# usamireko/WFL-ASR

Hardware: AMD Instinct MI355X
Metric: audio_seconds_labeled_per_sec_per_node (higher is better)
Workload: dtype bf16; 1 GPU; BASELINE configs[1]: openai/whisper-base + 2 Conformer blocks, 16 x 30 s clips per GPU; clips_per_gpu=16, frames_per_clip=1500, tags=141, parallelism=clip-sharded dp1, launch=eager, batches_in_flight=2

## Files before the change

include/wfl_asr.h:

```cpp
#ifndef WFL_ASR_H
#define WFL_ASR_H

#include <stdint.h>

#ifdef __cplusplus
extern "C" {
#endif

typedef struct wfl_model wfl_model;

#define WFL_ENC_WHISPER 0
#define WFL_ENC_WAVLM 1
#define WFL_ENC_NONE 2

#define WFL_ABI_VERSION 2

typedef struct wfl_arch {
  int32_t abi_version;
  int32_t encoder_type;
  int32_t d_model;
  int32_t enc_layers;
  int32_t enc_heads;
  int32_t enc_ffn;
  int32_t n_mels;
// ... 45 lines not shown

int32_t wfl_set_average_languages(wfl_model* m, const int32_t* ids_host, int32_t n);

int32_t wfl_num_frames(const wfl_model* m, int32_t L);
int64_t wfl_workspace_bytes(const wfl_model* m, int32_t B, int32_t L);

#define WFL_LANG_NONE 0
#define WFL_LANG_IDS 1
#define WFL_LANG_AVERAGE 2

int32_t wfl_forward(wfl_model* m, const float* wav, int64_t ldw, const int32_t* lens, int32_t B, int32_t L,
                    const int32_t* lang_id, int32_t lang_mode, float threshold, void* workspace,
                    int64_t workspace_bytes, int32_t* ids, int32_t* argmax, float* maxprob, float* offsets,
                    float* logits, float* hidden, int32_t* status, void* stream);

int32_t wfl_encode(wfl_model* m, const float* wav, int64_t ldw, const int32_t* lens, int32_t B, int32_t L, void* workspace,
                   int64_t workspace_bytes, float* hidden, void* stream);
int64_t wfl_head_workspace_bytes(const wfl_model* m, int32_t B, int32_t T);
int32_t wfl_head(wfl_model* m, const float* hidden, int32_t B, int32_t T, const int32_t* lang_id, int32_t lang_mode,
                 float threshold, void* workspace, int64_t workspace_bytes, int32_t* ids, int32_t* argmax, float* maxprob,
                 float* offsets, float* logits, int32_t* status, void* stream);

int32_t wfl_check(wfl_model* m, void* workspace, int64_t workspace_bytes, int32_t B, int32_t L, void* stream);


int32_t wfl_logmel(wfl_model* m, const float* wav, int64_t ldw, const int32_t* lens, int32_t B, int32_t L,
                   float* out, void* workspace, int64_t workspace_bytes, void* stream);

int32_t wfl_op_gemm(const void* A, int64_t lda, int32_t cin, int64_t tap_stride, const void* W, int32_t M, int32_t N,
                    int32_t K, int32_t n_valid, int32_t P, int32_t T, void* C, int64_t ldc, int64_t c_lead,
                    int32_t c_pitch, const float* bias, const void* res, int64_t ldres, float alpha, int32_t act,
                    int32_t glu, int32_t out_f32, void* stream);

int32_t wfl_op_gemm_split(const void* A_hi, const void* A_lo, int64_t lda, int32_t cin, int64_t tap_stride, const void* W3, int32_t M,
                          int32_t N, int32_t K, int32_t n_valid, int32_t P, int32_t T, void* C, void* C_lo, int64_t ldc,
                          int64_t c_lead, int32_t c_pitch, const float* bias, const void* res, const void* res_lo, int64_t ldres,
                          float alpha, int32_t act, int32_t glu, void* stream);

int32_t wfl_op_gemm_ln(const void* A, int64_t lda, const void* W, int32_t M, int32_t N, int32_t K, int32_t n_valid, int32_t P,
                       int32_t T, void* C, int64_t ldc, int64_t c_lead, int32_t c_pitch, const float* bias, const float* ln_s,
                       float ln_eps, int32_t act, void* stream);

int32_t wfl_op_attention(const void* QK, int64_t ldqk, int64_t lead, const void* V, int64_t ldv, void* O, int64_t ldo, int32_t B,
                         int32_t T, int32_t P, int32_t heads, int32_t d, void* stream);

int32_t wfl_op_attention_ex(const void* QK, const void* QK_lo, int64_t ldqk, int64_t lead, const void* V, const void* V_lo, int64_t ldv,
                            void* O, void* O_lo, int64_t ldo, int32_t B, int32_t T, int32_t P, int32_t heads, int32_t d, const float* bias,
                            const float* gate, const int32_t* clip_T, void* O8, void* O8_lo, int64_t ldo8, float o8_scale, int32_t* status,
                            void* stream);

int32_t wfl_op_relpos_table(const float* rel_emb, const int32_t* bucket_of_delta, int32_t max_t, int32_t heads, int32_t T, float* table,
                            void* stream);

int32_t wfl_op_relpos_gate(const void* x, const void* x_lo, int64_t ldx, int64_t lead, int32_t B, int32_t P, int32_t T, int32_t heads,
                           int32_t hd, const float* w8, const float* b8, const float* cst, float* gate, void* stream);

int32_t wfl_op_regroup(const void* x, int32_t d, int32_t groups, int32_t cpg, int64_t R, int64_t lead, int32_t B, int32_t P, int32_t T,
                       const int32_t* clip_T, void* xg, void* stream);

int32_t wfl_op_wav_stats(const float* wav, int64_t ldw, const int32_t* lens, int32_t B, int32_t L, double* stats, void* stream);

int32_t wfl_op_clip_frames(const int32_t* lens, int32_t B, int32_t L, int32_t n, const int32_t* kernel, const int32_t* stride,
                           int32_t min_len, int32_t* out, void* stream);

int64_t wfl_op_conv0_scratch_bytes(int32_t B, int32_t T0, int32_t C);
int32_t wfl_op_conv0(const float* wav, int64_t ldw, const int32_t* lens, int32_t B, int32_t L, const double* wstats, const float* w,
// ... 200 lines not shown
```

wfl-asr_amd/_lib.py:

```python
from __future__ import annotations

import ctypes as C
import os

import numpy as np

PKG = os.path.dirname(os.path.abspath(__file__))
LIB_PATH = os.environ.get("WFL_LIB_PATH") or os.path.join(PKG, "libwfl_asr_hip.so")
ABI_VERSION = 2


class WflArch(C.Structure):
    _fields_ = [
        ("abi_version", C.c_int32), ("encoder_type", C.c_int32), ("d_model", C.c_int32), ("enc_layers", C.c_int32),
        ("enc_heads", C.c_int32), ("enc_ffn", C.c_int32), ("n_mels", C.c_int32), ("max_positions", C.c_int32),
        ("num_classes", C.c_int32), ("o_id", C.c_int32), ("num_languages", C.c_int32), ("lang_emb_dim", C.c_int32),
        ("enable_bilstm", C.c_int32), ("bilstm_layers", C.c_int32), ("n_conformer", C.c_int32),
        ("conformer_heads", C.c_int32), ("conformer_ff_expansion", C.c_int32), ("conformer_kernel", C.c_int32),
        ("enable_dilated", C.c_int32), ("dilated_depth", C.c_int32), ("dilated_kernel", C.c_int32),
        ("wavlm_n_conv", C.c_int32), ("wavlm_conv_dim", C.c_int32 * 8), ("wavlm_conv_kernel", C.c_int32 * 8),
        ("wavlm_conv_stride", C.c_int32 * 8), ("wavlm_group_norm", C.c_int32), ("wavlm_conv_bias", C.c_int32),
        ("wavlm_stable_layer_norm", C.c_int32), ("wavlm_pos_conv_kernel", C.c_int32),
        ("wavlm_pos_conv_groups", C.c_int32), ("wavlm_num_buckets", C.c_int32), ("wavlm_max_distance", C.c_int32),
        ("wavlm_do_normalize", C.c_int32), ("fp8_weights", C.c_int32), ("mel_hop", C.c_int32), ("precision", C.c_int32), ("fp8_activations", C.c_int32),
        ("mel_sample_rate", C.c_int32), ("reserved", C.c_int32 * 5),
    ]


_P = C.c_void_p
_I = C.c_int32
_L = C.c_int64
_F = C.c_float

SIGNATURES = {
    "wfl_last_error": (C.c_char_p, []),
    "wfl_abi_version": (_I, []),
    "wfl_create": (_I, [C.POINTER(WflArch), C.POINTER(_P)]),
    "wfl_destroy": (None, [_P]),
    "wfl_load_tensor": (_I, [_P, C.c_char_p, _P, C.POINTER(_L), _I]),
    "wfl_finalize": (_I, [_P]),
    "wfl_num_frames": (_I, [_P, _I]),
    "wfl_workspace_bytes": (_L, [_P, _I, _I]),
    "wfl_device": (_I, [_P]),
    "wfl_set_average_languages": (_I, [_P, _P, _I]),
    "wfl_forward": (_I, [_P, _P, _L, _P, _I, _I, _P, _I, _F, _P, _L, _P, _P, _P, _P, _P, _P, _P, _P]),
    "wfl_encode": (_I, [_P, _P, _L, _P, _I, _I, _P, _L, _P, _P]),
    "wfl_head_workspace_bytes": (_L, [_P, _I, _I]),
    "wfl_head": (_I, [_P, _P, _I, _I, _P, _I, _F, _P, _L, _P, _P, _P, _P, _P, _P, _P]),
    "wfl_check": (_I, [_P, _P, _L, _I, _I, _P]),
    "wfl_logmel": (_I, [_P, _P, _L, _P, _I, _I, _P, _P, _L, _P]),
    "wfl_op_gemm": (_I, [_P, _L, _I, _L, _P, _I, _I, _I, _I, _I, _I, _P, _L, _L, _I, _P, _P, _L, _F, _I, _I, _I, _P]),
    "wfl_op_gemm_split": (_I, [_P, _P, _L, _I, _L, _P, _I, _I, _I, _I, _I, _I, _P, _P, _L, _L, _I, _P, _P, _P, _L, _F, _I, _I, _P]),
    "wfl_op_gemm_ln": (_I, [_P, _L, _P, _I, _I, _I, _I, _I, _I, _P, _L, _L, _I, _P, _P, _F, _I, _P]),
    "wfl_op_gemm_mx": (_I, [_P, _P, _L, _P, _P, _P, _F, _I, _I, _I, _I, _I, _P, _L, _L, _I, _P, _P, _P, _P, _F, _I, _P, _P, _L, _F, _P, _P]),
    "wfl_op_rows_fp8": (_I, [_P, _L, _P, _P, _P, _F, _L, _I, _I, _I, _I, _P, _P, _L, _P, _P]),
    "wfl_op_attention": (_I, [_P, _L, _L, _P, _L, _P, _L, _I, _I, _I, _I, _I, _P]),
    "wfl_op_attention_ex": (_I, [_P, _P, _L, _L, _P, _P, _L, _P, _P, _L, _I, _I, _I, _I, _I, _P, _P, _P, _P, _P, _L, _F, _P, _P]),
    "wfl_op_relpos_table": (_I, [_P, _P, _I, _I, _I, _P, _P]),
    "wfl_op_relpos_gate": (_I, [_P, _P, _L, _L, _I, _I, _I, _I, _I, _P, _P, _P, _P, _P]),
    "wfl_op_regroup": (_I, [_P, _I, _I, _I, _L, _L, _I, _I, _I, _P, _P, _P]),
    "wfl_op_wav_stats": (_I, [_P, _L, _P, _I, _I, _P, _P]),
    "wfl_op_clip_frames": (_I, [_P, _I, _I, _I, _P, _P, _I, _P, _P]),
    "wfl_op_conv0_scratch_bytes": (_L, [_I, _I, _I]),
    "wfl_op_conv0": (_I, [_P, _L, _P, _I, _I, _P, _P, _P, _P, _P, _I, _I, _P, _P, _L, _I, _I, _P, _L, _P]),
    "wfl_op_posconv": (_I, [_P, _L, _L, _I, _I, _I, _I, _I, _I, _P, _L, _P, _P, _P, _P, _P, _L, _P, _P]),
    "wfl_op_layernorm_act": (_I, [_P, _P, _L, _P, _P, _L, _P, _P, _F, _L, _I, _I, _I, _I, _I, _I, _P, _P]),
    "wfl_op_layernorm_pair": (_I, [_P, _P, _P, _P, _P, _P, _L, _P, _P, _P, _P, _F, _L, _I, _I, _I, _I, _I, _P, _P]),
    "wfl_op_layernorm": (_I, [_P, _L, _P, _L, _P, _P, _F, _L, _I, _I, _I, _I, _P]),
    "wfl_op_tag_decide": (_I, [_P, _L, _I, _I, _F, _I, _P, _P, _P, _P]),
    "wfl_host_median_filter": (_I, [_P, _I, _I, _P]),
    "wfl_host_decode_bio": (_I, [_P, _I, _P, _I, _P, _P, _I, C.c_double, _P, _P, _P, _I]),
    "wfl_host_merge_segments": (_I, [_P, _P, _P, _I, _I]),
    "wfl_host_format_lab": (_L, [_P, _P, _P, _I, _P, _I, _P, _L]),
    "wfl_host_load_wav": (_I, [C.c_char_p, _P, _L, _P, _P]),
    "wfl_host_load_wavs": (_I, [_P, _I, _P, _L, _L, _P, _P, _P, _I]),
    "wfl_host_load_wav_chunks": (_I, [C.c_char_p, _I, _L, _P, _L, _I, _P, _P, _P]),
    "wfl_host_read_pcm16": (_I, [_P, _I, _P, _L, _L, _P, _P, _P, _P, _I]),
    "wfl_resample_workspace_bytes": (_L, [_I, _I]),
    "wfl_resample_pcm16": (_I, [_P, _L, _P, _P, _I, _I, _I, _P, _L, _I, _P, _L, _P]),
    "wfl_boundary_workspace_bytes": (_L, [_I, _I]),
    "wfl_boundary_features": (_I, [_P, _L, _P, _I, _I, _P, _P, _P, _P, _P, _L, _P]),
    "wfl_align_workspace_bytes": (_L, [_P, _P, _I]),
    "wfl_align": (_I, [_P, _L, _I, _I, _P, _P, _P, _P, _P, _P, _I, _P, _L, _P, _P, _P, _P, _P]),
    "wfl_align_windowed": (_I, [_P, _L, _I, _I, _P, _P, _P, _P, _P, _P, _P, _I, _P, _L, _P, _P, _P, _P, _P]),
# ... 87 lines not shown
```

wfl-asr_amd/csrc/gemm_stream.hip:

```cpp
#include "common.h"
#include <cstdlib>
#include <cstring>
#include <type_traits>

#define SBK 32
#ifndef SNST
#define SNST 4
#endif

#ifndef SNCU
#define SNCU 256
#endif

typedef __attribute__((address_space(1))) const void* sgptr_t;
typedef __attribute__((address_space(3))) void* slptr_t;
typedef __attribute__((ext_vector_type(2))) __bf16 bf16x2;

static __device__ __forceinline__ void sglds(const bf16_t* g, char* l) {
  __builtin_amdgcn_global_load_lds((sgptr_t)g, (slptr_t)l, 16, 0, 0);
}
static __device__ __forceinline__ int sswz(int row) { return (-(row >> 2)) & 3; }
static __device__ __forceinline__ int xswz(int row) { return ((row >> 2) & 1) << 1; }
#define XROT_ROWS 223
template <int N>
static __device__ __forceinline__ void wait_vm() { asm volatile("s_waitcnt vmcnt(%0)" ::"n"(N) : "memory"); }

#ifdef WFL_GEMM_STAMPS
#define SSTAMP(k) do { if (tid == 0 && p.stamps) { p.stamps[(long)blockIdx.x * 8 + (k)] = __builtin_amdgcn_s_memrealtime(); \
    if ((k) == 1) p.stamps[(long)blockIdx.x * 8 + 5] = __builtin_amdgcn_s_memtime(); \
    if ((k) == 2) p.stamps[(long)blockIdx.x * 8 + 6] = __builtin_amdgcn_s_memtime(); } } while (0)
#else
#define SSTAMP(k) do { } while (0)
#endif

template <int ACT, int MT, bool RES, int LNF, bool STATS, bool CONV, bool W8 = false, bool A8 = false, bool OUT8 = false, bool NOLO = false, bool ROT = false>
__global__ __launch_bounds__(512) void gemm_stream_kernel(GemmArgs p) {
  static_assert(!NOLO || CONV, "only the conv mode has an optional low half");
  static_assert(!ROT || CONV, "only the conv mode rotates frame fragments");
  static_assert(!CONV || (MT == 6 && !RES && LNF == 0 && !STATS), "conv mode: 192-row tiles, plain epilogue");
  static_assert(!W8 || (!CONV && MT == 6), "fp8 weights: plain 192-row mode");
  static_assert(!A8 || (!W8 && !CONV && MT == 6 && LNF == 0 && !STATS), "fp8 x fp8: the plain 192-row mode, no LayerNorm folding");
  static_assert(!OUT8 || (A8 && !RES), "fp8 output: the fp8 x fp8 kernel, no residual");
  constexpr int BMV = MT * 32;
#ifdef WFL_LAB_STB32
  constexpr int STB = 512 * SBK * 2;
  constexpr int WOFF = 256 * SBK * 2;
#else
  constexpr int STB = CONV ? 256 * SBK * 2 : BMV * SBK * 2 + 256 * SBK * (W8 ? 1 : 2);
  constexpr int WOFF = CONV ? 0 : BMV * SBK * 2;
#endif
  constexpr int AEXT = 224 * SBK * 2;
  constexpr int AOFF = SNST * STB;
  constexpr bool LOUT = RES || (CONV && !NOLO);
  constexpr int NSTORE = (LOUT ? 4 : 2) * MT + (STATS ? MT : 0);
  constexpr int SROW = 4;
  extern __shared__ __attribute__((aligned(16))) char smem[];
  float* stat_lds = (float*)(smem + SNST * STB + (CONV ? 2 * AEXT : 0));
  const int tid = threadIdx.x;
  const int lane = tid & 63;
  const int wid = __builtin_amdgcn_readfirstlane(tid >> 6);
  const int grp = wid >> 2, wq = wid & 3;
  const int g = lane >> 4, c = lane & 15;
  const int G = gridDim.x;

  SSTAMP(0);
  const int tiles_n = p.N / 256;
  const int tiles_m = (p.M + BMV - 1) / BMV;
  const int ntiles = tiles_m * tiles_n;
  const int nk = p.K / SBK;
  auto tile_of = [&](int v, int& m0, int& n0) __attribute__((always_inline)) {
    const int q = ntiles >> 3, r = ntiles & 7, x = v & 7, i = v >> 3;
    const int bid = (x < r ? x * (q + 1) : r * (q + 1) + (x - r) * q) + i;
    const int tm = bid / tiles_n;
    m0 = tm * BMV;
    n0 = (bid - tm * tiles_n) * 256;
  };
  const int wm = grp * (MT * 16), wn = wq * 64;

  const bool two_x = CONV ? wid < 6 : (MT == 8 || wid < 4);
  const int xg0 = CONV ? (wid < 6 ? wid * 2 : 12 + (wid - 6)) : ((MT == 8 || wid < 4) ? wid * 2 : 8 + (wid - 4));
  const int ntaps = CONV ? (p.tap_wrap > 0 ? p.tap_wrap : p.K / p.cin) : 1;
  const int nchunk = CONV ? p.cin / SBK : 1;
  const bf16_t* a_src[2];
  const bf16_t* w_src[2];
  const char* w8_src = nullptr;
  int pv = blockIdx.x, pkt = 0, issued = 0;
  int islot = 0;
// ... 96 lines not shown
  };
  auto prefetch_one = [&]() __attribute__((always_inline)) {
    if (pv >= ntiles) return;
    issue_stage();
    if (pkt == nk) {
      pkt = 0; ptap_k = 0; pbase = 0; pcc = 0; ptap = 0; ptap_i = 0; pseg = 0; pa_off = 0; pw_off = 0;
      pv += G;
      if (pv < ntiles) set_src(pv);
    }
  };
  auto wait_stage = [&](int need, bool with_stores) __attribute__((always_inline)) {
    const int younger = issued - need - 1;
    if (younger < 0) return;
    constexpr int L2X = CONV ? 2 : (W8 ? 3 : 4), L1X = CONV ? 2 : (W8 ? 2 : 3);
    static_assert(SNST >= 3 && SNST <= 6, "ring depth");
#define WFL_WAITY(L)                                                                              \
    do {                                                                                          \
      if (SNST >= 6 && younger >= 4) { if (with_stores) wait_vm<4 * (L) + NSTORE>(); else wait_vm<4 * (L)>(); }       \
      else if (SNST >= 5 && younger >= 3) { if (with_stores) wait_vm<3 * (L) + NSTORE>(); else wait_vm<3 * (L)>(); }  \
      else if (younger >= 2) { if (with_stores) wait_vm<2 * (L) + NSTORE>(); else wait_vm<2 * (L)>(); }              \
      else if (younger == 1) { if (with_stores) wait_vm<(L) + NSTORE>(); else wait_vm<(L)>(); }                      \
      else { if (with_stores) wait_vm<NSTORE>(); else wait_vm<0>(); }                                                \
    } while (0)
    if (CONV || two_x) WFL_WAITY(L2X); else WFL_WAITY(L1X);
#undef WFL_WAITY
  };

  int w_off[4];
#pragma unroll
  for (int v = 0; v < 4; ++v) {
#ifdef WFL_LAB_NOPERM
    const int r = wn + 16 * v + c;
#else
    const int r = wn + 32 * (v >> 1) + 8 * (c >> 2) + 4 * (v & 1) + (c & 3);
#endif
    w_off[v] = W8 ? WOFF + (r >> 3) * 256 + ((((r & 7) * 4 + g) ^ (((r >> 3) & 1) << 1) ^ (((r >> 4) & 1) << 4)) << 3)
                  : WOFF + r * 64 + ((g ^ sswz(r)) << 4);
  }
  const int x_off = wm * 64 + c * 64 + ((g ^ sswz(c)) << 4);

  f32x4 acc[MT][4];
#pragma unroll
  for (int u = 0; u < MT; ++u)
#pragma unroll
    for (int v = 0; v < 4; ++v) acc[u][v] = (f32x4){0.f, 0.f, 0.f, 0.f};
  float sa1 = 0.f, sa2 = 0.f, sb1 = 0.f, sb2 = 0.f;

  auto epilogue = [&](int m0, int n0) __attribute__((always_inline)) {
    const int nb = n0 + wn + 8 * g;
    constexpr int FCOL = ROT ? MT : 1, FROW = ROT ? 1 : 16;
    int mrow0 = m0 + wm + FCOL * c;
    int sidx_w = (((grp * 4 + wq) * (MT * 16)) + c) * 2, sidx_g = ((grp * 4 * (MT * 16)) + c) * 2, sidx_l = (grp * (MT * 16) + c) * 2;
    asm volatile("" : "+v"(mrow0), "+v"(sidx_w), "+v"(sidx_g), "+v"(sidx_l));
    f32x4 bj[4], sj[4], cj[(W8 || A8) ? 4 : 1];
#pragma unroll
    for (int h = 0; h < 2; ++h)
#pragma unroll
      for (int q = 0; q < 2; ++q) {
#ifdef WFL_ABL_EPI_NOLOAD
        bj[2 * h + q] = (f32x4){0.f, 0.f, 0.f, 0.f};
        if (LNF) sj[2 * h + q] = (f32x4){1.f, 1.f, 1.f, 1.f};
        if (W8 || A8) cj[2 * h + q] = (f32x4){1.f, 1.f, 1.f, 1.f};
#else
        bj[2 * h + q] = p.bias ? *(const f32x4*)(p.bias + nb + 32 * h + 4 * q) : (f32x4){0.f, 0.f, 0.f, 0.f};
        if (LNF) sj[2 * h + q] = *(const f32x4*)(p.ln_s + nb + 32 * h + 4 * q);
        if (W8 || A8) cj[2 * h + q] = *(const f32x4*)(p.w8_scale + nb + 32 * h + 4 * q);
#endif
      }
    float sa[A8 ? MT : 1];
    if (A8) {
#pragma unroll
      for (int u = 0; u < MT; ++u) {
        int m = mrow0 + FROW * u;
        m = m < p.M ? m : p.M - 1;
        sa[u] = p.a8_scale ? p.a8_scale[p.a8_lead + m] : p.a8_static;
      }
    }
    int P_ = p.P, cpitch = p.c_pitch;
    asm volatile("" : "+s"(P_), "+s"(cpitch));
    const float invP = __builtin_amdgcn_rcpf((float)P_);
    int orow[MT];
#pragma unroll
    for (int u = 0; u < MT; ++u) {
      const int m = mrow0 + FROW * u;
      int b = (int)((float)m * invP);
      int t = m - b * P_;
      if (t < 0) { t += P_; --b; }
      if (t >= P_) { t -= P_; ++b; }
      orow[u] = (m < p.M && t < p.T) ? (int)p.c_lead + b * cpitch + t : -1;
    }
    if (p.clip_T) {
#pragma unroll
      for (int u = 0; u < MT; ++u)
        if (orow[u] >= 0) {
          const int m = mrow0 + FROW * u;
          int b = (int)((float)m * invP);
          int t = m - b * P_;
          if (t < 0) { t += P_; --b; }
          if (t >= P_) { t -= P_; ++b; }
          if (t >= p.clip_T[b]) orow[u] = -1;
        }
    }
    constexpr int RING = 3;
    bf16x8 rr[RES ? RING : 1][2], rl[RES ? RING : 1][2];
    const bf16_t* res_lo = p.res_lo ? p.res_lo : p.res;
    const float lo_scale = p.res_lo ? 1.f : 0.f;
    auto load_res = [&](int u, int slot) __attribute__((always_inline)) {
      const long r = orow[u] >= 0 ? orow[u] : p.c_lead;
#pragma unroll
      for (int h = 0; h < 2; ++h) {
#ifdef WFL_ABL_EPI_NOLOAD
        rr[slot][h] = (bf16x8){0, 0, 0, 0, 0, 0, 0, 0}; rl[slot][h] = rr[slot][h]; (void)r;
#else
        rr[slot][h] = *(const bf16x8*)(p.res + r * p.ldres + nb + 32 * h);
        rl[slot][h] = *(const bf16x8*)(res_lo + r * p.ldres + nb + 32 * h);
#endif
      }
    };
    if (RES) {
#pragma unroll
      for (int u = 0; u < RING && u < MT; ++u) load_res(u, u);
    }
    float mu[LNF ? MT : 1], rs[LNF ? MT : 1];
    if (LNF == 1) {
#pragma unroll
      for (int u = 0; u < MT; ++u) {
        const float2 s = *(const float2*)(stat_lds + sidx_l + u * 32);
        mu[u] = s.x;
        rs[u] = s.y;
      }
    }
    if (LNF == 2) {
      f32x4 sp[MT][2];
#pragma unroll
      for (int u = 0; u < MT; ++u) {
        int m = mrow0 + FROW * u;
        m = m < p.M ? m : p.M - 1;
        const f32x4* q = (const f32x4*)(p.stats_in + (p.stats_lead + m) * (2 * SROW));
        sp[u][0] = q[0];
        sp[u][1] = q[1];
      }
#pragma unroll
      for (int u = 0; u < MT; ++u) {
        float a1 = sp[u][0][0], a2 = sp[u][0][1];
        if (p.stats_nsl > 1) { a1 += sp[u][0][2]; a2 += sp[u][0][3]; }
        if (p.stats_nsl > 2) { a1 += sp[u][1][0]; a2 += sp[u][1][1]; }
        if (p.stats_nsl > 3) { a1 += sp[u][1][2]; a2 += sp[u][1][3]; }
        float mean, ex2;
        if (p.ln_k_pow2) { mean = a1 * p.ln_inv_k; ex2 = a2 * p.ln_inv_k; }
        else { mean = a1 / (float)p.K; ex2 = a2 / (float)p.K; }
        mu[u] = mean;
        rs[u] = rsqrtf(fmaxf(__builtin_fmaf(-mean, mean, ex2), 0.f) + p.ln_eps);
      }
    }
    char* trash = (char*)p.trash + lane * 16;
#ifdef WFL_ABL_EPI_NOSTORE
#define WFL_KEEP(k) false
#else
#define WFL_KEEP(k) (k)
#endif
    float t1 = 0.f, t2 = 0.f;
    float amax8 = 0.f;
#pragma unroll
    for (int u = 0; u < MT; ++u) {
      __builtin_amdgcn_sched_barrier(0);
#pragma unroll
      for (int h = 0; h < 2; ++h) {
        float x[8];
#pragma unroll
        for (int q = 0; q < 2; ++q)
#pragma unroll
          for (int e = 0; e < 4; ++e) {
            float v = acc[u][2 * h + q][e];
            if (W8 || A8) v *= cj[2 * h + q][e];
            if (A8) v *= sa[u];
            if (LNF) v = (v - mu[u] * sj[2 * h + q][e]) * rs[u];
            if (ACT == WFL_ACT_GELU) {
              x[4 * q + e] = v + bj[2 * h + q][e];
              if (e & 1) {
                const f32x2 y = gelu_erf2((f32x2){x[4 * q + e - 1], x[4 * q + e]});
                x[4 * q + e - 1] = y[0]; x[4 * q + e] = y[1];
              }
              continue;
            }
            v = apply_act<ACT>(v + bj[2 * h + q][e]);
            if (RES) v = (bf2f(rr[u % RING][h][4 * q + e]) + lo_scale * bf2f(rl[u % RING][h][4 * q + e])) + p.alpha * v;
            x[4 * q + e] = v;
          }
        bf16x8 o;
#pragma unroll
        for (int e = 0; e < 8; ++e) o[e] = f2bf(x[e]);
        const bool keep = orow[u] >= 0 && nb + 32 * h < p.n_valid;
        if (OUT8) {
          int w0 = 0, w1 = 0;
          const float keepf = keep ? 1.f : 0.f;
#pragma unroll
          for (int e = 0; e < 8; ++e) {
            const float y = x[e] * p.c8_inv_scale;
            amax8 = fmaxf(amax8, fabsf(y) * keepf);
            x[e] = fminf(fmaxf(y, -448.f), 448.f);
          }
          w0 = __builtin_amdgcn_cvt_pk_fp8_f32(x[0], x[1], w0, false); w0 = __builtin_amdgcn_cvt_pk_fp8_f32(x[2], x[3], w0, true);
          w1 = __builtin_amdgcn_cvt_pk_fp8_f32(x[4], x[5], w1, false); w1 = __builtin_amdgcn_cvt_pk_fp8_f32(x[6], x[7], w1, true);
          char* d8 = (char*)(p.c8 + (long)orow[u] * p.ldc8 + nb + 32 * h);
          d8 = WFL_KEEP(keep) ? d8 : trash;
          *(uint2*)d8 = make_uint2((unsigned)w0, (unsigned)w1);
          continue;
        }
        char* dst = (char*)((bf16_t*)p.C + (long)orow[u] * p.ldc + nb + 32 * h);
        dst = WFL_KEEP(keep) ? dst : trash;
        *(bf16x8*)dst = o;
        if (LOUT) {
          bf16x8 ol;
#pragma unroll
          for (int e = 0; e < 8; ++e) ol[e] = f2bf(x[e] - bf2f(o[e]));
          char* dl = (char*)(p.c_lo + (long)orow[u] * p.ldc + nb + 32 * h);
          dl = WFL_KEEP(keep && p.c_lo) ? dl : trash;
          *(bf16x8*)dl = ol;
        }
        if (STATS) {
#pragma unroll
          for (int e = 0; e < 8; ++e) { const float r = bf2f(o[e]); t1 += r; t2 = fmaf(r, r, t2); }
        }
      }
      if (STATS) {
        t1 += __shfl_xor(t1, 16); t2 += __shfl_xor(t2, 16);
        t1 += __shfl_xor(t1, 32); t2 += __shfl_xor(t2, 32);
        if (g == 0) *(float2*)(stat_lds + sidx_w + u * 32) = float2{t1, t2};
        t1 = t2 = 0.f;
      }
#pragma unroll
      for (int v = 0; v < 4; ++v) acc[u][v] = (f32x4){0.f, 0.f, 0.f, 0.f};
      if (RES && u + RING < MT) load_res(u + RING, u % RING);
    }
    if (OUT8 && p.err) {
      if (__builtin_amdgcn_ballot_w64(amax8 > 448.f) && lane == 0) atomicOr(p.err, 2u);
    }
    if (STATS) {
      unsigned* cnt = (unsigned*)(stat_lds + 8 * (MT * 16) * 2) + grp;
      __builtin_amdgcn_s_waitcnt(0xC07F);
      unsigned ticket = 0;
      if (lane == 0) ticket = atomicAdd(cnt, 1u);
      ticket = __builtin_amdgcn_readfirstlane(ticket);
      const bool last = ticket == 3;
      if (last && lane == 0) *cnt = 0;
#pragma unroll
      for (int u = 0; u < MT; ++u) {
        float a1 = 0.f, a2 = 0.f;
#pragma unroll
        for (int w4 = 0; w4 < 4; ++w4) {
          const float2 v = *(const float2*)(stat_lds + sidx_g + w4 * (MT * 32) + u * 32);
          a1 += v.x; a2 += v.y;
        }
        float* sd = p.stats_out + ((long)orow[u] * SROW + (n0 >> 8)) * 2;
        sd = (last && orow[u] >= 0 && g == 0) ? sd : (float*)trash;
        *(float2*)sd = float2{a1, a2};
      }
    }
  };

  if (STATS && tid < 2) ((unsigned*)(stat_lds + 8 * (MT * 16) * 2))[tid] = 0;
#pragma unroll
  for (int t = 0; t < SNST - 1; ++t) prefetch_one();
  wait_stage(0, false);
  __builtin_amdgcn_s_barrier();
  SSTAMP(1);
// ... 149 lines not shown
        if (CONV) issue_stage(); else issue_stage_split(ndc_c);
#else
        ++issued; ++pkt; if (CONV) { if (++ptap == ntaps) { ptap = 0; ++pcc; ++pccg; } }
#endif
        if (GRP1) wait_vm<(SNST - 2) * NL - NDC>();
        __builtin_amdgcn_s_waitcnt(0xC07F);
        __builtin_amdgcn_s_barrier();
        SSB();
        mma_all(ndc_c);
        SSB();
        if (!GRP1) wait_vm<(SNST - 2) * NL>();
        __builtin_amdgcn_s_barrier();
        SSB();
        ++s;
        rslot = rslot + 1 == SNST ? 0 : rslot + 1;
      }
    };
    step_general(0, std::true_type{});
#pragma unroll
    for (int kt = 1; kt < SNST - 2; ++kt) step_general(kt, std::false_type{});
    if (grp) steps_steady(std::true_type{}); else steps_steady(std::false_type{});
    for (int kt = nk - SNST > SNST - 2 ? nk - SNST : SNST - 2; kt < nk; ++kt) step_general(kt, std::false_type{});
    pm0 = m0; pn0 = n0;
    have_prev = true;
  }
  SSTAMP(2);
  SSTAMP(3);
  if (have_prev) epilogue(pm0, pn0);
  if (LNF == 1 && !grp) __builtin_amdgcn_s_barrier();
  SSTAMP(4);
#undef SSB
}

template <int ACT, int MT, bool RES, int LNF, bool STATS, bool CONV = false, bool W8 = false, bool A8 = false, bool OUT8 = false, bool NOLO = false, bool ROT = false>
static int launch_stream(const GemmArgs& a, hipStream_t s) {
  constexpr int BMV = MT * 32;
#ifdef WFL_LAB_STB32
  constexpr int lds = SNST * 512 * SBK * 2 + 8 * (MT * 16) * 2 * 4 + 64;
#else
  constexpr int lds = (CONV ? SNST * 256 * SBK * 2 + 2 * 224 * SBK * 2 : SNST * (BMV * SBK * 2 + 256 * SBK * (W8 ? 1 : 2))) + 8 * (MT * 16) * 2 * 4 + 64;
#endif
  const int tiles = ((a.M + BMV - 1) / BMV) * (a.N / 256);
  auto k = gemm_stream_kernel<ACT, MT, RES, LNF, STATS, CONV, W8, A8, OUT8, NOLO, ROT>;
  static WflOncePerDevice attr_once;
  if (attr_once.need()) {
    if (hipFuncSetAttribute((const void*)k, hipFuncAttributeMaxDynamicSharedMemorySize, lds) != hipSuccess) return -2;
  }
  g_wfl_gemm_kernel_id = CONV ? 6 : ((W8 || A8) ? 7 : (MT == 6 ? 1 : 5));
  hipLaunchKernelGGL(k, dim3(tiles < SNCU ? tiles : SNCU), dim3(512), lds, s, a);
  return hipGetLastError() == hipSuccess ? 0 : -3;
}

template <int ACT, bool RES, int LNF, bool STATS = false>
static int launch_stream_mt(const GemmArgs& a, hipStream_t s) {
  static int forced = -1;
  if (forced < 0) { const char* e = getenv("WFL_GEMM_BM"); forced = e ? atoi(e) : 0; }
#ifdef WFL_STREAM_MT8
  if (forced == 256) return launch_stream<ACT, 8, RES, LNF, STATS>(a, s);
#endif
  return launch_stream<ACT, 6, RES, LNF, STATS>(a, s);
}

static bool wfl_gemm_stream_conv(const GemmArgs& a) {
  static int off = -1;
  if (off < 0) { const char* e = getenv("WFL_GEMM_NO_CONV"); off = e && atoi(e) ? 1 : 0; }
  if (off) return false;
  const int taps = a.tap_wrap > 0 ? a.tap_wrap : a.K / a.cin;
  if (a.tap_wrap > 0 && a.K != 3 * a.tap_wrap * a.cin) return false;
  return a.cin < a.K && a.K % a.cin == 0 && taps <= 32 && taps >= SNST - 1 && a.tap_stride == a.lda && a.cin % SBK == 0 &&
         !a.res && !a.ln_s && !a.stats_out;
}

bool wfl_gemm_stream_conv_takes(const GemmArgs& a);

template <bool ROT>
static int launch_conv(const GemmArgs& g, hipStream_t s) {
  if (!g.c_lo) {
    switch (g.act) {
      case WFL_ACT_NONE: return launch_stream<WFL_ACT_NONE, 6, false, 0, false, true, false, false, false, true, ROT>(g, s);
      case WFL_ACT_GELU: return launch_stream<WFL_ACT_GELU, 6, false, 0, false, true, false, false, false, true, ROT>(g, s);
      case WFL_ACT_RELU: return launch_stream<WFL_ACT_RELU, 6, false, 0, false, true, false, false, false, true, ROT>(g, s);
    }
    return 1;
  }
  switch (g.act) {
    case WFL_ACT_NONE: return launch_stream<WFL_ACT_NONE, 6, false, 0, false, true, false, false, false, false, ROT>(g, s);
    case WFL_ACT_GELU: return launch_stream<WFL_ACT_GELU, 6, false, 0, false, true, false, false, false, false, ROT>(g, s);
    case WFL_ACT_RELU: return launch_stream<WFL_ACT_RELU, 6, false, 0, false, true, false, false, false, false, ROT>(g, s);
  }
  return 1;
}
bool wfl_gemm_stream_takes(const GemmArgs& a) {
  static int off = -1;
  if (off < 0) { const char* e = getenv("WFL_GEMM_NO_STREAM"); off = e && atoi(e) ? 1 : 0; }
  if (off) return false;
#ifdef WFL_LAB_NOSTREAM
  return false;
#endif
  if (a.glu || a.out_f32 || a.pos || a.clip_bias) return false;
  if (a.a8 >= 2) return false;
  if (a.tap_wrap > 0 && (a.ln_s || a.w8_scale || a.a8)) return false;
  if (a.c_lo && !a.res && !wfl_gemm_stream_conv(a)) return false;
  if (a.w8_scale && (a.cin < a.K || a.K % 64)) return false;
  if (a.a8 && (!a.w8_scale || a.ln_s || a.stats_out || a.stats_in || a.K % 128 || a.lda % 16 || a.K / 64 < 8 || (a.c8 && (a.res || a.ldc8 % 8))))
    return false;
  if (a.c8 && !a.a8) return false;
  if (a.N % 256 || a.K % SBK || a.cin % SBK || a.K / SBK < 8 || a.n_valid % 8) return false;
  if (a.stats_out && (!a.res || a.N / 256 > 4)) return false;
  if (a.stats_in && (!a.ln_s || a.stats_nsl <= 0 || a.stats_nsl > 4)) return false;
  if (a.res && a.act != WFL_ACT_NONE) return false;
  if (a.ln_s && (a.res || a.cin < a.K || (a.act != WFL_ACT_NONE && a.act != WFL_ACT_GELU))) return false;
  if (a.act == WFL_ACT_SIGMOID) return false;
  return true;
}


bool wfl_gemm_stream_conv_takes(const GemmArgs& a) { return wfl_gemm_stream_takes(a) && wfl_gemm_stream_conv(a); }

int wfl_launch_gemm_stream(const GemmArgs& a, hipStream_t s) {
  if (!wfl_gemm_stream_takes(a)) return 1;
  static void* trash[32] = {nullptr};
  int dev = 0;
  (void)hipGetDevice(&dev);
  dev &= 31;
  if (!trash[dev]) {
    if (hipMalloc(&trash[dev], 4096) != hipSuccess) return -2;
  }
  GemmArgs g = a;
  g.trash = trash[dev];
  g.ln_k_pow2 = (g.K & (g.K - 1)) == 0;
  g.ln_inv_k = g.ln_k_pow2 ? 1.0f / (float)g.K : 0.f;
  if (g.a8) {
    g.K /= 2; g.cin = g.K; g.lda /= 2;
    if (g.c8) return g.act == WFL_ACT_GELU ? launch_stream<WFL_ACT_GELU, 6, false, 0, false, false, false, true, true>(g, s) : -1;
    if (g.res) return g.act == WFL_ACT_NONE ? launch_stream<WFL_ACT_NONE, 6, true, 0, false, false, false, true>(g, s) : -1;
    if (g.act == WFL_ACT_NONE) return launch_stream<WFL_ACT_NONE, 6, false, 0, false, false, false, true>(g, s);
    return -1;
  }
  if (g.w8_scale) {
    if (g.ln_s && g.stats_in) {
      if (g.act == WFL_ACT_NONE) return launch_stream<WFL_ACT_NONE, 6, false, 2, false, false, true>(g, s);
      if (g.act == WFL_ACT_GELU) return launch_stream<WFL_ACT_GELU, 6, false, 2, false, false, true>(g, s);
      return -1;
    }
    if (g.res && !g.ln_s && g.act == WFL_ACT_NONE)
      return g.stats_out ? launch_stream<WFL_ACT_NONE, 6, true, 0, true, false, true>(g, s)
                         : launch_stream<WFL_ACT_NONE, 6, true, 0, false, false, true>(g, s);
    if (!g.res && !g.ln_s) {
      if (g.act == WFL_ACT_NONE) return launch_stream<WFL_ACT_NONE, 6, false, 0, false, false, true>(g, s);
      if (g.act == WFL_ACT_GELU) return launch_stream<WFL_ACT_GELU, 6, false, 0, false, false, true>(g, s);
    }
    return -1;
  }
  if (g.ln_s) {
    if (g.stats_in) {
      switch (g.act) {
        case WFL_ACT_NONE: return launch_stream_mt<WFL_ACT_NONE, false, 2>(g, s);
        case WFL_ACT_GELU: return launch_stream_mt<WFL_ACT_GELU, false, 2>(g, s);
      }
      return 1;
    }
    switch (g.act) {
      case WFL_ACT_NONE: return launch_stream_mt<WFL_ACT_NONE, false, 1>(g, s);
      case WFL_ACT_GELU: return launch_stream_mt<WFL_ACT_GELU, false, 1>(g, s);
    }
    return 1;
  }
  if (wfl_gemm_stream_conv(g)) {
    const char* e = getenv("WFL_CONV_ROTATE");
    const bool rot = !(e && e[0] == '0' && !e[1]);
    return rot ? launch_conv<true>(g, s) : launch_conv<false>(g, s);
  }
  if (g.res) return g.stats_out ? launch_stream_mt<WFL_ACT_NONE, true, 0, true>(g, s) : launch_stream_mt<WFL_ACT_NONE, true, 0>(g, s);
  switch (g.act) {
    case WFL_ACT_NONE: return launch_stream_mt<WFL_ACT_NONE, false, 0>(g, s);
    case WFL_ACT_GELU: return launch_stream_mt<WFL_ACT_GELU, false, 0>(g, s);
    case WFL_ACT_RELU: return launch_stream_mt<WFL_ACT_RELU, false, 0>(g, s);
  }
  return 1;
}
```

wfl-asr_amd/csrc/model.hip:

```cpp
#include "common.h"
#include "../../include/wfl_asr.h"

#include <cmath>
#include <cstdint>
#include <cstdio>
#include <cstring>
#include <map>
#include <set>
#include <string>
#include <vector>

int wfl_launch_logmel(const LogmelArgs& a, bf16_t* out, long ldo, long lead, int P, float* ref_out, hipStream_t s, bf16_t* out_lo = nullptr);
int wfl_launch_precise_finish(const PreciseFinishArgs& a, hipStream_t s);
int wfl_launch_melpower(const LogmelArgs& a, int hop, bf16_t* out, long ldo, long lead, int P, int split, int shift, hipStream_t s);

int wfl_launch_tag_decide(const TagArgs& a, hipStream_t s);
int wfl_launch_f32_to_rows(const float* in, bf16_t* x, long ldx, long lead, int B, int P, int T, int C, hipStream_t s, int split,
                           int shift, bf16_t* x_lo = nullptr);

int wfl_launch_lstm(LstmArgs a, void* exchange, hipStream_t s);

int wfl_launch_wav_stats(const float* wav, long ldw, int B, int L, double* stats, hipStream_t s, const int* lens = nullptr);
int wfl_launch_conv0(const Conv0Args& a, int group_norm, hipStream_t s);
int wfl_launch_clip_frames(const int* lens, int B, int L, int n, const int* kernel, const int* stride, int min_len, int* out, hipStream_t s);
// ... 1955 lines not shown
                       int32_t c_pitch, const float* bias, const void* res, const void* res_lo, void* c_lo, float alpha, int32_t act,
                       void* c8, void* c8_lo, int64_t ldc8, float c8_inv_scale, int32_t* status, void* stream) {
  GemmArgs g{};
  g.A = (const bf16_t*)A8; g.a8_lo = (const unsigned char*)A8_lo; g.a8 = A8_lo ? 3 : 2; g.lda = lda; g.cin = K; g.W = (const bf16_t*)W8;
  g.w8_scale = w_scale; g.a8_scale = a_scale; g.a8_static = a_static; g.a8_lead = 0;
  g.M = M; g.N = N; g.K = K; g.n_valid = N; g.P = P; g.T = T; g.C = C; g.ldc = ldc; g.c_lead = c_lead; g.c_pitch = c_pitch;
  g.bias = bias; g.res = (const bf16_t*)res; g.res_lo = (const bf16_t*)res_lo; g.c_lo = (bf16_t*)c_lo; g.ldres = ldc; g.alpha = alpha; g.act = act;
  g.c8 = (unsigned char*)c8; g.c8_lo = (unsigned char*)c8_lo; g.ldc8 = ldc8; g.c8_inv_scale = c8_inv_scale; g.err = (unsigned*)status;
  if (!A8 || !W8 || !w_scale || (!C && !c8) || M <= 0 || P <= 0 || P % 8) return fail(-1, "wfl_op_gemm_mx: bad argument");
  const int r = wfl_launch_gemm_mx(g, (hipStream_t)stream);
  return r ? fail(r == 1 ? -1 : r, "wfl_op_gemm_mx: shape or argument not taken by gemm_mx.hip (" + std::to_string(r) + ")") : 0;
}

int32_t wfl_op_rows_fp8(const void* x, int64_t ldx, const void* x_lo, const float* gamma, const float* beta, float eps, int64_t lead,
                        int32_t B, int32_t P, int32_t T, int32_t C, void* y8, void* y8_lo, int64_t ldy8, float* scale, void* stream) {
  const int r = wfl_launch_rows_fp8((const bf16_t*)x, ldx, (const bf16_t*)x_lo, gamma, beta, eps, lead, B, P, T, C, (unsigned char*)y8, ldy8,
                                    scale, (hipStream_t)stream, (unsigned char*)y8_lo);
  return r ? fail(r, "wfl_op_rows_fp8: invalid arguments or launch failure") : 0;
}

int32_t wfl_op_gemm(const void* A, int64_t lda, int32_t cin, int64_t tap_stride, const void* W, int32_t M, int32_t N,
                    int32_t K, int32_t n_valid, int32_t P, int32_t T, void* C, int64_t ldc, int64_t c_lead, int32_t c_pitch,
                    const float* bias, const void* res, int64_t ldres, float alpha, int32_t act, int32_t glu,
                    int32_t out_f32, void* stream) {
  GemmArgs g{};
  g.A = (const bf16_t*)A; g.lda = lda; g.cin = cin > 0 ? cin : K; g.tap_stride = tap_stride;
  g.W = (const bf16_t*)W; g.M = M; g.N = N; g.K = K; g.n_valid = n_valid; g.P = P; g.T = T;
  g.C = C; g.ldc = ldc; g.c_lead = c_lead; g.c_pitch = c_pitch; g.bias = bias;
  g.res = (const bf16_t*)res; g.ldres = ldres; g.alpha = alpha; g.act = act; g.glu = glu; g.out_f32 = out_f32;
  const int r = wfl_launch_gemm(g, (hipStream_t)stream);
  return r ? fail(r, "wfl_op_gemm: invalid arguments or launch failure (" + std::to_string(r) + ")") : 0;
}

int32_t wfl_op_gemm_ln(const void* A, int64_t lda, const void* W, int32_t M, int32_t N, int32_t K, int32_t n_valid, int32_t P,
                       int32_t T, void* C, int64_t ldc, int64_t c_lead, int32_t c_pitch, const float* bias, const float* ln_s,
                       float ln_eps, int32_t act, void* stream) {
  if (!ln_s) return fail(-1, "wfl_op_gemm_ln: ln_s is required");
  GemmArgs g{};
  g.A = (const bf16_t*)A; g.lda = lda; g.cin = K; g.tap_stride = 0;
  g.W = (const bf16_t*)W; g.M = M; g.N = N; g.K = K; g.n_valid = n_valid; g.P = P; g.T = T;
  g.C = C; g.ldc = ldc; g.c_lead = c_lead; g.c_pitch = c_pitch; g.bias = bias; g.alpha = 1.f; g.act = act;
  g.ln_s = ln_s; g.ln_eps = ln_eps;
  const int r = wfl_launch_gemm(g, (hipStream_t)stream);
  return r ? fail(r, "wfl_op_gemm_ln: shape not supported by the LayerNorm-folding kernel or launch failure (" + std::to_string(r) + ")") : 0;
}

int32_t wfl_op_gemm_split(const void* A_hi, const void* A_lo, int64_t lda, int32_t cin, int64_t tap_stride, const void* W3, int32_t M,
                          int32_t N, int32_t K, int32_t n_valid, int32_t P, int32_t T, void* C, void* C_lo, int64_t ldc, int64_t c_lead,
                          int32_t c_pitch, const float* bias, const void* res, const void* res_lo, int64_t ldres, float alpha,
                          int32_t act, int32_t glu, void* stream) {
  if (!A_hi || !A_lo || !W3 || !C || !C_lo) return fail(-1, "wfl_op_gemm_split: null argument");
  if (K <= 0 || (cin > 0 && K % cin)) return fail(-1, "wfl_op_gemm_split: K must be a whole number of taps");
  GemmArgs g{};
  g.A = (const bf16_t*)A_hi; g.lda = lda; g.cin = cin > 0 ? cin : K; g.tap_stride = tap_stride;
  g.tap_wrap = K / g.cin; g.seg_off = (long)((const bf16_t*)A_lo - (const bf16_t*)A_hi);
  g.W = (const bf16_t*)W3; g.M = M; g.N = N; g.K = 3 * K; g.n_valid = n_valid; g.P = P; g.T = T;
  g.C = C; g.c_lo = (bf16_t*)C_lo; g.ldc = ldc; g.c_lead = c_lead; g.c_pitch = c_pitch; g.bias = bias;
  g.res = (const bf16_t*)res; g.res_lo = res ? (const bf16_t*)res_lo : nullptr; g.ldres = ldres; g.alpha = alpha; g.act = act; g.glu = glu;
  g.ln_eps = 1e-5f;
  const int r = wfl_launch_gemm(g, (hipStream_t)stream);
  return r ? fail(r, "wfl_op_gemm_split: invalid arguments or launch failure (" + std::to_string(r) + ")") : 0;
}

int32_t wfl_op_attention(const void* QK, int64_t ldqk, int64_t lead, const void* V, int64_t ldv, void* O, int64_t ldo, int32_t B, int32_t T,
                         int32_t P, int32_t heads, int32_t d, void* stream) {
  AttnArgs a{};
// ... 176 lines not shown
```

Baseline: 131,300 audio-s/s.

## Route GLU, fp32, positional and per-clip-bias epilogue GEMMs through the stream kernel

Adds an EPI template parameter to the streaming GEMM kernel so it can emit fp32 output, add a positional embedding after GELU, fuse GLU gating, or add a per-clip bias in its epilogue. GEMMs carrying these epilogues used to be rejected by the stream path and fell back to another GEMM kernel. They can now use the streaming kernel when M is at least 2048 and the other conditions hold. The price is extra template instantiations and more complex epilogue code, including a different weight-row permutation for GLU that could introduce correctness risk.

```diff
diff --git a/include/wfl_asr.h b/include/wfl_asr.h
--- a/include/wfl_asr.h
+++ b/include/wfl_asr.h
@@ -101,6 +101,11 @@
                     int32_t c_pitch, const float* bias, const void* res, int64_t ldres, float alpha, int32_t act,
                     int32_t glu, int32_t out_f32, void* stream);
 
+int32_t wfl_op_gemm_epi(const void* A, int64_t lda, int32_t cin, int64_t tap_stride, const void* W, int32_t M, int32_t N, int32_t K,
+                        int32_t n_valid, int32_t P, int32_t T, void* C, void* C_lo, int64_t ldc, int64_t c_lead, int32_t c_pitch,
+                        const float* bias, const void* pos, int64_t ldpos, const float* clip_bias, const int32_t* clip_idx,
+                        int32_t clip_ld, int32_t act, void* stream);
+
 int32_t wfl_op_gemm_split(const void* A_hi, const void* A_lo, int64_t lda, int32_t cin, int64_t tap_stride, const void* W3, int32_t M,
                           int32_t N, int32_t K, int32_t n_valid, int32_t P, int32_t T, void* C, void* C_lo, int64_t ldc,
                           int64_t c_lead, int32_t c_pitch, const float* bias, const void* res, const void* res_lo, int64_t ldres,
diff --git a/wfl-asr_amd/_lib.py b/wfl-asr_amd/_lib.py
--- a/wfl-asr_amd/_lib.py
+++ b/wfl-asr_amd/_lib.py
@@ -50,6 +50,7 @@
     "wfl_check": (_I, [_P, _P, _L, _I, _I, _P]),
     "wfl_logmel": (_I, [_P, _P, _L, _P, _I, _I, _P, _P, _L, _P]),
     "wfl_op_gemm": (_I, [_P, _L, _I, _L, _P, _I, _I, _I, _I, _I, _I, _P, _L, _L, _I, _P, _P, _L, _F, _I, _I, _I, _P]),
+    "wfl_op_gemm_epi": (_I, [_P, _L, _I, _L, _P, _I, _I, _I, _I, _I, _I, _P, _P, _L, _L, _I, _P, _P, _L, _P, _P, _I, _I, _P]),
     "wfl_op_gemm_split": (_I, [_P, _P, _L, _I, _L, _P, _I, _I, _I, _I, _I, _I, _P, _P, _L, _L, _I, _P, _P, _P, _L, _F, _I, _I, _P]),
     "wfl_op_gemm_ln": (_I, [_P, _L, _P, _I, _I, _I, _I, _I, _I, _P, _L, _L, _I, _P, _P, _F, _I, _P]),
     "wfl_op_gemm_mx": (_I, [_P, _P, _L, _P, _P, _P, _F, _I, _I, _I, _I, _I, _P, _L, _L, _I, _P, _P, _P, _P, _F, _I, _P, _P, _L, _F, _P, _P]),
diff --git a/wfl-asr_amd/csrc/gemm_stream.hip b/wfl-asr_amd/csrc/gemm_stream.hip
--- a/wfl-asr_amd/csrc/gemm_stream.hip
+++ b/wfl-asr_amd/csrc/gemm_stream.hip
@@ -33,8 +33,16 @@
 #define SSTAMP(k) do { } while (0)
 #endif
 
-template <int ACT, int MT, bool RES, int LNF, bool STATS, bool CONV, bool W8 = false, bool A8 = false, bool OUT8 = false, bool NOLO = false, bool ROT = false>
+#define EPI_NONE 0
+#define EPI_F32 1
+#define EPI_POS 2
+#define EPI_GLU 3
+#define EPI_CLIP 4
+template <int ACT, int MT, bool RES, int LNF, bool STATS, bool CONV, bool W8 = false, bool A8 = false, bool OUT8 = false, bool NOLO = false, bool ROT = false,
+          int EPI = EPI_NONE>
 __global__ __launch_bounds__(512) void gemm_stream_kernel(GemmArgs p) {
+  static_assert(EPI == EPI_NONE || (MT == 6 && !RES && LNF == 0 && !STATS && !CONV && !W8 && !A8), "epilogue kinds: the plain 192-row bf16 mode");
+  static_assert((EPI != EPI_F32 && EPI != EPI_GLU && EPI != EPI_CLIP) || ACT == WFL_ACT_NONE, "fp32 output, GLU and the per-clip bias come without an activation");
   static_assert(!NOLO || CONV, "only the conv mode has an optional low half");
   static_assert(!ROT || CONV, "only the conv mode rotates frame fragments");
   static_assert(!CONV || (MT == 6 && !RES && LNF == 0 && !STATS), "conv mode: 192-row tiles, plain epilogue");
@@ -51,8 +59,8 @@
 #endif
   constexpr int AEXT = 224 * SBK * 2;
   constexpr int AOFF = SNST * STB;
-  constexpr bool LOUT = RES || (CONV && !NOLO);
-  constexpr int NSTORE = (LOUT ? 4 : 2) * MT + (STATS ? MT : 0);
+  constexpr bool LOUT = RES || (CONV && !NOLO) || EPI == EPI_POS || EPI == EPI_CLIP;
+  constexpr int NSTORE = ((LOUT || EPI == EPI_F32) ? 4 : 2) * MT + (STATS ? MT : 0);
   constexpr int SROW = 4;
   extern __shared__ __attribute__((aligned(16))) char smem[];
   float* stat_lds = (float*)(smem + SNST * STB + (CONV ? 2 * AEXT : 0));
@@ -215,7 +223,7 @@
 #ifdef WFL_LAB_NOPERM
     const int r = wn + 16 * v + c;
 #else
-    const int r = wn + 32 * (v >> 1) + 8 * (c >> 2) + 4 * (v & 1) + (c & 3);
+    const int r = EPI == EPI_GLU ? wn + 16 * v + c : wn + 32 * (v >> 1) + 8 * (c >> 2) + 4 * (v & 1) + (c & 3);
 #endif
     w_off[v] = W8 ? WOFF + (r >> 3) * 256 + ((((r & 7) * 4 + g) ^ (((r >> 3) & 1) << 1) ^ (((r >> 4) & 1) << 4)) << 3)
                   : WOFF + r * 64 + ((g ^ sswz(r)) << 4);
@@ -245,7 +253,7 @@
         if (LNF) sj[2 * h + q] = (f32x4){1.f, 1.f, 1.f, 1.f};
         if (W8 || A8) cj[2 * h + q] = (f32x4){1.f, 1.f, 1.f, 1.f};
 #else
-        bj[2 * h + q] = p.bias ? *(const f32x4*)(p.bias + nb + 32 * h + 4 * q) : (f32x4){0.f, 0.f, 0.f, 0.f};
+        bj[2 * h + q] = p.bias ? *(const f32x4*)(p.bias + (EPI == EPI_GLU ? n0 + wn + 16 * (2 * h + q) + 4 * g : nb + 32 * h + 4 * q)) : (f32x4){0.f, 0.f, 0.f, 0.f};
         if (LNF) sj[2 * h + q] = *(const f32x4*)(p.ln_s + nb + 32 * h + 4 * q);
         if (W8 || A8) cj[2 * h + q] = *(const f32x4*)(p.w8_scale + nb + 32 * h + 4 * q);
 #endif
@@ -263,6 +271,9 @@
     asm volatile("" : "+s"(P_), "+s"(cpitch));
     const float invP = __builtin_amdgcn_rcpf((float)P_);
     int orow[MT];
+    int trow[EPI == EPI_POS ? MT : 1];
+    int crow[EPI == EPI_CLIP ? MT : 1];
+    const int blast = EPI == EPI_CLIP ? (p.M - 1) / P_ : 0;
 #pragma unroll
     for (int u = 0; u < MT; ++u) {
       const int m = mrow0 + FROW * u;
@@ -271,6 +282,12 @@
       if (t < 0) { t += P_; --b; }
       if (t >= P_) { t -= P_; ++b; }
       orow[u] = (m < p.M && t < p.T) ? (int)p.c_lead + b * cpitch + t : -1;
+      if (EPI == EPI_POS) trow[u] = t < p.T ? t : 0;
+      if (EPI == EPI_CLIP) crow[u] = m < p.M ? b : blast;
+    }
+    if (EPI == EPI_CLIP) {
+#pragma unroll
+      for (int u = 0; u < MT; ++u) crow[u] = p.clip_idx[crow[u]] * p.clip_ld;
     }
     if (p.clip_T) {
 #pragma unroll
@@ -285,10 +302,16 @@
         }
     }
     constexpr int RING = 3;
-    bf16x8 rr[RES ? RING : 1][2], rl[RES ? RING : 1][2];
+    constexpr bool RINGED = RES || EPI == EPI_POS;
+    bf16x8 rr[RINGED ? RING : 1][2], rl[RES ? RING : 1][2];
     const bf16_t* res_lo = p.res_lo ? p.res_lo : p.res;
     const float lo_scale = p.res_lo ? 1.f : 0.f;
     auto load_res = [&](int u, int slot) __attribute__((always_inline)) {
+      if (EPI == EPI_POS) {
+#pragma unroll
+        for (int h = 0; h < 2; ++h) rr[slot][h] = *(const bf16x8*)(p.pos + (long)trow[u] * p.ldpos + (nb + 32 * h < p.n_valid ? nb + 32 * h : 0));
+        return;
+      }
       const long r = orow[u] >= 0 ? orow[u] : p.c_lead;
 #pragma unroll
       for (int h = 0; h < 2; ++h) {
@@ -300,9 +323,19 @@
 #endif
       }
     };
-    if (RES) {
+    if (RINGED) {
 #pragma unroll
       for (int u = 0; u < RING && u < MT; ++u) load_res(u, u);
+    }
+    constexpr int CRING = 2;
+    f32x4 cbv[EPI == EPI_CLIP ? CRING : 1][4];
+    auto load_cb = [&](int u, int slot) __attribute__((always_inline)) {
+#pragma unroll
+      for (int j = 0; j < 4; ++j) cbv[slot][j] = *(const f32x4*)(p.clip_bias + crow[u] + nb + 32 * (j >> 1) + 4 * (j & 1));
+    };
+    if (EPI == EPI_CLIP) {
+#pragma unroll
+      for (int u = 0; u < CRING && u < MT; ++u) load_cb(u, u);
     }
     float mu[LNF ? MT : 1], rs[LNF ? MT : 1];
     if (LNF == 1) {
@@ -347,6 +380,22 @@
 #pragma unroll
     for (int u = 0; u < MT; ++u) {
       __builtin_amdgcn_sched_barrier(0);
+      if (EPI == EPI_GLU) {
+#pragma unroll
+        for (int jp = 0; jp < 2; ++jp) {
+          bf16x4 o;
+#pragma unroll
+          for (int e = 0; e < 4; ++e) o[e] = f2bf((acc[u][2 * jp][e] + bj[2 * jp][e]) * sigmoidf_(acc[u][2 * jp + 1][e] + bj[2 * jp + 1][e]));
+          const int col = ((n0 + wn) >> 1) + 16 * jp + 4 * g;
+          const bool keep = orow[u] >= 0 && col < (p.n_valid >> 1);
+          char* dst = (char*)((bf16_t*)p.C + (long)orow[u] * p.ldc + col);
+          dst = WFL_KEEP(keep) ? dst : trash;
+          *(bf16x4*)dst = o;
+        }
+#pragma unroll
+        for (int v = 0; v < 4; ++v) acc[u][v] = (f32x4){0.f, 0.f, 0.f, 0.f};
+        continue;
+      }
 #pragma unroll
       for (int h = 0; h < 2; ++h) {
         float x[8];
@@ -367,9 +416,34 @@
               continue;
             }
             v = apply_act<ACT>(v + bj[2 * h + q][e]);
+            if (EPI == EPI_CLIP) v += cbv[u % CRING][2 * h + q][e];
             if (RES) v = (bf2f(rr[u % RING][h][4 * q + e]) + lo_scale * bf2f(rl[u % RING][h][4 * q + e])) + p.alpha * v;
             x[4 * q + e] = v;
           }
+        if (EPI == EPI_POS) {
+#pragma unroll
+          for (int e = 0; e < 8; ++e) x[e] += bf2f(rr[u % RING][h][e]);
+        }
+        if (EPI == EPI_F32) {
+          float* const row = (float*)p.C + (long)orow[u] * p.ldc;
+#pragma unroll
+          for (int q = 0; q < 2; ++q) {
+            const int col = nb + 32 * h + 4 * q;
+            char* d4 = (char*)(row + col);
+            d4 = WFL_KEEP(orow[u] >= 0 && col + 4 <= p.n_valid) ? d4 : trash;
+            *(f32x4*)d4 = (f32x4){x[4 * q], x[4 * q + 1], x[4 * q + 2], x[4 * q + 3]};
+            const int dcol = (p.n_valid & ~3) - (n0 + wn + 32 * h + 4 * q);
+            if ((p.n_valid & 3) && dcol >= 0 && dcol < 32 && !(dcol & 7)) {
+#pragma unroll
+              for (int e = 0; e < 3; ++e) {
+                char* d1 = (char*)(row + col + e);
+                d1 = WFL_KEEP(orow[u] >= 0 && col == (p.n_valid & ~3) && col + e < p.n_valid) ? d1 : trash;
+                *(float*)d1 = x[4 * q + e];
+              }
+            }
+          }
+          continue;
+        }
         bf16x8 o;
 #pragma unroll
         for (int e = 0; e < 8; ++e) o[e] = f2bf(x[e]);
@@ -414,7 +488,8 @@
       }
 #pragma unroll
       for (int v = 0; v < 4; ++v) acc[u][v] = (f32x4){0.f, 0.f, 0.f, 0.f};
-      if (RES && u + RING < MT) load_res(u + RING, u % RING);
+      if (RINGED && u + RING < MT) load_res(u + RING, u % RING);
+      if (EPI == EPI_CLIP && u + CRING < MT) load_cb(u + CRING, u % CRING);
     }
     if (OUT8 && p.err) {
       if (__builtin_amdgcn_ballot_w64(amax8 > 448.f) && lane == 0) atomicOr(p.err, 2u);
@@ -630,7 +705,8 @@
 #undef SSB
 }
 
-template <int ACT, int MT, bool RES, int LNF, bool STATS, bool CONV = false, bool W8 = false, bool A8 = false, bool OUT8 = false, bool NOLO = false, bool ROT = false>
+template <int ACT, int MT, bool RES, int LNF, bool STATS, bool CONV = false, bool W8 = false, bool A8 = false, bool OUT8 = false, bool NOLO = false, bool ROT = false,
+          int EPI = EPI_NONE>
 static int launch_stream(const GemmArgs& a, hipStream_t s) {
   constexpr int BMV = MT * 32;
 #ifdef WFL_LAB_STB32
@@ -639,7 +715,7 @@
   constexpr int lds = (CONV ? SNST * 256 * SBK * 2 + 2 * 224 * SBK * 2 : SNST * (BMV * SBK * 2 + 256 * SBK * (W8 ? 1 : 2))) + 8 * (MT * 16) * 2 * 4 + 64;
 #endif
   const int tiles = ((a.M + BMV - 1) / BMV) * (a.N / 256);
-  auto k = gemm_stream_kernel<ACT, MT, RES, LNF, STATS, CONV, W8, A8, OUT8, NOLO, ROT>;
+  auto k = gemm_stream_kernel<ACT, MT, RES, LNF, STATS, CONV, W8, A8, OUT8, NOLO, ROT, EPI>;
   static WflOncePerDevice attr_once;
   if (attr_once.need()) {
     if (hipFuncSetAttribute((const void*)k, hipFuncAttributeMaxDynamicSharedMemorySize, lds) != hipSuccess) return -2;
@@ -688,6 +764,23 @@
   }
   return 1;
 }
+static int wfl_gemm_stream_epi(const GemmArgs& a) {
+  const int kind = a.glu ? EPI_GLU : (a.out_f32 ? EPI_F32 : (a.pos ? EPI_POS : (a.clip_bias ? EPI_CLIP : EPI_NONE)));
+  if ((a.glu != 0) + (a.out_f32 != 0) + (a.pos != nullptr) + (a.clip_bias != nullptr) != 1) return EPI_NONE;
+  if (const char* e = getenv("WFL_STREAM_EPI")) {
+    static const char* const names[] = {"", "f32", "pos", "glu", "clip"};
+    if (!strstr(e, names[kind])) return EPI_NONE;
+  }
+  if (a.M < 2048 || a.tap_wrap > 0 || a.w8_scale || a.a8 || a.c8 || a.ln_s || a.res || a.stats_out || a.stats_in || wfl_gemm_stream_conv(a)) return EPI_NONE;
+  switch (kind) {
+    case EPI_F32: return (!a.acc_f32 && a.act == WFL_ACT_NONE && a.ldc % 4 == 0) ? kind : EPI_NONE;
+    case EPI_POS: return a.act == WFL_ACT_GELU ? kind : EPI_NONE;
+    case EPI_GLU: return (a.act == WFL_ACT_NONE && !a.c_lo) ? kind : EPI_NONE;
+    case EPI_CLIP: return (a.act == WFL_ACT_NONE && a.clip_idx) ? kind : EPI_NONE;
+  }
+  return EPI_NONE;
+}
+
 bool wfl_gemm_stream_takes(const GemmArgs& a) {
   static int off = -1;
   if (off < 0) { const char* e = getenv("WFL_GEMM_NO_STREAM"); off = e && atoi(e) ? 1 : 0; }
@@ -695,15 +788,16 @@
 #ifdef WFL_LAB_NOSTREAM
   return false;
 #endif
-  if (a.glu || a.out_f32 || a.pos || a.clip_bias) return false;
+  const int epi = wfl_gemm_stream_epi(a);
+  if ((a.glu || a.out_f32 || a.pos || a.clip_bias) && epi == EPI_NONE) return false;
   if (a.a8 >= 2) return false;
   if (a.tap_wrap > 0 && (a.ln_s || a.w8_scale || a.a8)) return false;
-  if (a.c_lo && !a.res && !wfl_gemm_stream_conv(a)) return false;
+  if (a.c_lo && !a.res && epi != EPI_POS && epi != EPI_CLIP && !wfl_gemm_stream_conv(a)) return false;
   if (a.w8_scale && (a.cin < a.K || a.K % 64)) return false;
   if (a.a8 && (!a.w8_scale || a.ln_s || a.stats_out || a.stats_in || a.K % 128 || a.lda % 16 || a.K / 64 < 8 || (a.c8 && (a.res || a.ldc8 % 8))))
     return false;
   if (a.c8 && !a.a8) return false;
-  if (a.N % 256 || a.K % SBK || a.cin % SBK || a.K / SBK < 8 || a.n_valid % 8) return false;
+  if (a.N % 256 || a.K % SBK || a.cin % SBK || a.K / SBK < 8 || (a.n_valid % 8 && epi != EPI_F32)) return false;
   if (a.stats_out && (!a.res || a.N / 256 > 4)) return false;
   if (a.stats_in && (!a.ln_s || a.stats_nsl <= 0 || a.stats_nsl > 4)) return false;
   if (a.res && a.act != WFL_ACT_NONE) return false;
@@ -750,6 +844,12 @@
     }
     return -1;
   }
+  switch (wfl_gemm_stream_epi(g)) {
+    case EPI_F32: return launch_stream<WFL_ACT_NONE, 6, false, 0, false, false, false, false, false, false, false, EPI_F32>(g, s);
+    case EPI_POS: return launch_stream<WFL_ACT_GELU, 6, false, 0, false, false, false, false, false, false, false, EPI_POS>(g, s);
+    case EPI_GLU: return launch_stream<WFL_ACT_NONE, 6, false, 0, false, false, false, false, false, false, false, EPI_GLU>(g, s);
+    case EPI_CLIP: return launch_stream<WFL_ACT_NONE, 6, false, 0, false, false, false, false, false, false, false, EPI_CLIP>(g, s);
+  }
   if (g.ln_s) {
     if (g.stats_in) {
       switch (g.act) {
diff --git a/wfl-asr_amd/csrc/model.hip b/wfl-asr_amd/csrc/model.hip
--- a/wfl-asr_amd/csrc/model.hip
+++ b/wfl-asr_amd/csrc/model.hip
@@ -2011,6 +2011,20 @@
   return r ? fail(r, "wfl_op_gemm: invalid arguments or launch failure (" + std::to_string(r) + ")") : 0;
 }
 
+int32_t wfl_op_gemm_epi(const void* A, int64_t lda, int32_t cin, int64_t tap_stride, const void* W, int32_t M, int32_t N, int32_t K,
+                        int32_t n_valid, int32_t P, int32_t T, void* C, void* C_lo, int64_t ldc, int64_t c_lead, int32_t c_pitch,
+                        const float* bias, const void* pos, int64_t ldpos, const float* clip_bias, const int32_t* clip_idx,
+                        int32_t clip_ld, int32_t act, void* stream) {
+  if (clip_bias && !clip_idx) return fail(-1, "wfl_op_gemm_epi: clip_bias needs clip_idx");
+  GemmArgs g{};
+  g.A = (const bf16_t*)A; g.lda = lda; g.cin = cin > 0 ? cin : K; g.tap_stride = tap_stride;
+  g.W = (const bf16_t*)W; g.M = M; g.N = N; g.K = K; g.n_valid = n_valid; g.P = P; g.T = T;
+  g.C = C; g.c_lo = (bf16_t*)C_lo; g.ldc = ldc; g.c_lead = c_lead; g.c_pitch = c_pitch; g.bias = bias; g.alpha = 1.f; g.act = act;
+  g.pos = (const bf16_t*)pos; g.ldpos = ldpos; g.clip_bias = clip_bias; g.clip_idx = clip_idx; g.clip_ld = clip_ld;
+  const int r = wfl_launch_gemm(g, (hipStream_t)stream);
+  return r ? fail(r, "wfl_op_gemm_epi: invalid arguments or launch failure (" + std::to_string(r) + ")") : 0;
+}
+
 int32_t wfl_op_gemm_ln(const void* A, int64_t lda, const void* W, int32_t M, int32_t N, int32_t K, int32_t n_valid, int32_t P,
                        int32_t T, void* C, int64_t ldc, int64_t c_lead, int32_t c_pitch, const float* bias, const float* ln_s,
                        float ln_eps, int32_t act, void* stream) {
```

Result: no change. 131,600 audio-s/s (median of 6 runs) (+0.2%).
